# AHupuJR/REFID

Measured on AMD Instinct MI355X. Metric: interpolated frames/sec (train step) GoPro 256x256 11+1, higher is better.
Workload: dtype f32

## Files before the change

refid_amd/csrc/conv_split.hip:

```cpp
#include "common.h"
#include "conv_args.h"
#include "conv_epilogue.h"
#include "conv_planes.h"

#ifndef REFID_SPLIT_ABLATE
#define REFID_SPLIT_ABLATE 0
#endif

namespace {

constexpr int F16_TGT = 8;
constexpr int F16_SLACK = 6;
constexpr int F16_E0 = F16_TGT + 1;
constexpr int TW = 32;
constexpr int KC = 8;
constexpr int NTH = 256;
__device__ __forceinline__ int cdiv_dev(int a, int b) { return (a + b - 1) / b; }

#ifdef REFID_SPLIT_TRACE
__device__ unsigned long long* g_split_trace = nullptr;
__device__ unsigned long long* g_split_ktrace = nullptr;
__device__ int g_split_ktrace_wg = -1;
#define SPLIT_STAMP(slot)                                                                    \
    do {                                                                                     \
        if (g_split_trace && threadIdx.x == 0) g_split_trace[(size_t)blockIdx.x * 8 + (slot)] = wall_clock64(); \
    } while (0)
#define SPLIT_KSTAMP(ch, slot)                                                               \
    do {                                                                                     \
        if (ktrace && (threadIdx.x & 63) == 0)                                               \
            g_split_ktrace[(((threadIdx.x >> 6) * 64 + ((ch) & 63)) * 8) + (slot)] = wall_clock64(); \
    } while (0)
#else
#define SPLIT_STAMP(slot) do {} while (0)
#define SPLIT_KSTAMP(ch, slot) do {} while (0)
#endif

template <int MT_, int NT_, int PL_, int KS_, int MODE_, bool F16_ = false>
struct SCfg {
    static constexpr int MT = MT_, NT = NT_, PL = PL_, KS = KS_;
    static constexpr int MODE = MODE_;
    static constexpr bool F16 = F16_;
    static constexpr int TH = 4 * MT, BN = 32 * NT;
    static constexpr int HWD = (MODE == 1) ? TW + 1 : TW + 2;
    static constexpr int NTAP = (MODE == 0) ? 10 : 4;
    static constexpr int NSTEP = NTAP / 2;
    static constexpr int HP = ((MODE == 1) ? TH + 1 : TH + 2) * HWD;
    static constexpr int A_SLOTS = HP;
    static constexpr int B_SLOTS = NTAP * BN;
    static constexpr int A_ITEMS = (A_SLOTS + NTH - 1) / NTH;
    static constexpr int B_ITEMS = (PL * B_SLOTS + NTH - 1) / NTH;
    static constexpr int C4 = BN / 4;
    static constexpr int XS = C4 + 1;
    static constexpr int LDS_LOOP = KS * PL * (A_SLOTS + B_SLOTS) * 16 + (F16 ? 16 : 0);
    static constexpr int LDS_EPI = 4 * 32 * XS * 16;
    static constexpr int LDS_BYTES = LDS_LOOP > LDS_EPI ? LDS_LOOP : LDS_EPI;
};

template <int MT, int NT, int PL, int KS, int MODE, bool F16 = false>
__global__ __launch_bounds__(NTH, 2) void conv_split_kernel(const ConvKArgs a) {
    using C = SCfg<MT, NT, PL, KS, MODE, F16>;
    static_assert(!F16 || PL == 2, "the fp16 form has two planes");
    constexpr int HP = C::HP, BN = C::BN, HWD = C::HWD, NTAP = C::NTAP, NSTEP = C::NSTEP;
    static_assert(MODE != 1 || KS == 2, "MODE 1: a stage = the two column positions of a block");
    extern __shared__ __attribute__((aligned(16))) char smem[];
    f32x4* sA = reinterpret_cast<f32x4*>(smem);
    f32x4* sB = sA + KS * PL * C::A_SLOTS;
    float* sM = reinterpret_cast<float*>(sB + KS * PL * C::B_SLOTS);

    const int tid = threadIdx.x;
    const int lane = tid & 63, wave = tid >> 6;
    const int li = lane & 31, kh = lane >> 5;

    const int xcd = blockIdx.x & 7, slot = blockIdx.x >> 3;
    int bt = (slot / a.ncot) * 8 + xcd;
    if (bt >= a.tilesX * a.tilesY * a.N) return;
    const int n0 = (slot % a.ncot) * BN;
    const int tx = bt % a.tilesX; bt /= a.tilesX;
    const int ty = bt % a.tilesY;
    const int n = bt / a.tilesY;
    const int oy0 = ty * C::TH, ox0 = tx * TW;
    SPLIT_STAMP(0);
#ifdef REFID_SPLIT_TRACE
    const bool ktrace = g_split_ktrace && (int)blockIdx.x == g_split_ktrace_wg;
    if (g_split_trace && tid == 0) {
        unsigned hw, xcc;
        asm volatile("s_getreg_b32 %0, hwreg(HW_REG_HW_ID)" : "=s"(hw));
        asm volatile("s_getreg_b32 %0, hwreg(HW_REG_XCC_ID)" : "=s"(xcc));
        g_split_trace[(size_t)blockIdx.x * 8 + 7] = ((unsigned long long)xcc << 32) | hw;
    }
#endif

    const int limA = (int)min((long long)a.N * a.H * a.W * a.ldA * 4, 0x7fffffffLL);
    const int limB = a.inB ? (int)min((long long)a.N * a.H * a.W * a.ldB * 4, 0x7fffffffLL) : 0;
    const int wChunk = PL * NTAP * a.CoutPad * 16;
    const int nsub = cdiv_dev(a.Ctot, KC) * (MODE == 1 ? 4 : 1);
    const int cls = (MODE == 2) ? blockIdx.y : 0;
    const int py = cls >> 1, px = cls & 1;
    const __amdgpu_buffer_rsrc_t rsW = __builtin_amdgcn_make_buffer_rsrc(
        reinterpret_cast<char*>(const_cast<float*>(a.w)) + (F16 ? PACK_HEADER_BYTES : 0) + (long long)cls * nsub * wChunk, 0,
        (int)min((long long)nsub * wChunk, 0x7fffffffLL), 0x00020000);
    const int eW = F16 ? *reinterpret_cast<const int*>(a.w) : 0;
    int eRef = F16_E0;
    int voA[C::A_ITEMS], voB[C::A_ITEMS], vo1x[2][MODE == 1 ? C::A_ITEMS : 1];
#pragma unroll
    for (int it = 0; it < C::A_ITEMS; ++it) {
        const int hp = tid + it * NTH;
        if constexpr (MODE == 1) {
            const int r0 = 2 * (oy0 + hp / HWD) - 1, c0 = 2 * (ox0 + hp % HWD) - 1;
#pragma unroll
            for (int sy = 0; sy < 2; ++sy)
#pragma unroll
                for (int sx = 0; sx < 2; ++sx) {
                    const int iy = r0 + sy, ix = c0 + sx;
                    const bool ok = hp < HP && iy >= 0 && iy < a.H && ix >= 0 && ix < a.W;
                    const int vo = ok ? ((n * a.H + iy) * a.W + ix) * a.ldA * 4 : OOB;
                    if (sx == 0) (sy ? voB[it] : voA[it]) = vo;
                    else vo1x[sy][it] = vo;
                }
        } else {
            const int iy = oy0 - 1 + hp / HWD, ix = ox0 - 1 + hp % HWD;
            const bool ok = hp < HP && iy >= 0 && iy < a.H && ix >= 0 && ix < a.W;
            const int pix = (n * a.H + iy) * a.W + ix;
            voA[it] = ok ? pix * a.ldA * 4 : OOB;
            voB[it] = ok ? pix * a.ldB * 4 : OOB;
        }
    }
    int voW[C::B_ITEMS];
#pragma unroll
    for (int it = 0; it < C::B_ITEMS; ++it) {
        const int s = tid + it * NTH;
        const int co = s % BN, r = s / BN;
        const int row = a.coBase + n0 + co;
        voW[it] = (s < PL * C::B_SLOTS && row < a.CoutPad) ? (r * a.CoutPad + row) * 16 : OOB;
    }

    f32x4 ra[KS][C::A_ITEMS][2], rb[KS][C::B_ITEMS];
    constexpr int NLD = 2 * C::A_ITEMS + C::B_ITEMS;
    auto load_part = [&](int chReal, int part) {
        const int ch = REFID_SPLIT_ABLATE == 3 ? 0 : chReal;
#pragma unroll
        for (int sub = 0; sub < KS; ++sub) {
            const int c0 = (MODE == 1 ? (ch >> 1) : (ch * KS + sub)) * KC;
            const bool fromA = MODE != 0 || c0 < a.Ca;
            const bool cok = c0 < a.Ctot;
            const int soff = (fromA ? c0 : c0 - a.Ca) * 4;
            const bool sy1 = MODE == 1 && (ch & 1);
            const __amdgpu_buffer_rsrc_t rs = __builtin_amdgcn_make_buffer_rsrc(
                const_cast<float*>(fromA ? a.inA : a.inB), 0, fromA ? limA : limB, 0x00020000);
#pragma unroll
            for (int i = 0; i < NLD; ++i) {
                if ((sub * NLD + i) * NSTEP / NLD != part && part >= 0) continue;
                if (i < 2 * C::A_ITEMS) {
                    const int it = i >> 1;
                    int vo;
                    if constexpr (MODE == 1) vo = sub == 0 ? (sy1 ? voB[it] : voA[it]) : (sy1 ? vo1x[1][it] : vo1x[0][it]);
                    else vo = fromA ? voA[it] : voB[it];
                    if (!cok) vo = OOB;
                    ra[sub][it][i & 1] = __builtin_bit_cast(f32x4, __builtin_amdgcn_raw_buffer_load_b128(rs, vo, soff + 16 * (i & 1), 0));
                } else {
                    const int it = i - 2 * C::A_ITEMS;
                    int vo = voW[it];
                    if constexpr (MODE == 2) vo |= (ch * KS + sub < nsub) ? 0 : OOB;
                    rb[sub][it] = __builtin_bit_cast(
                        f32x4, __builtin_amdgcn_raw_buffer_load_b128(rsW, vo, (ch * KS + sub) * wChunk, 0));
                }
            }
        }
    };
    auto load_chunk = [&](int ch) { load_part(ch, -1); };
    auto post_max = [&]() {
        float tm = 0.f;
#pragma unroll
        for (int sub = 0; sub < KS; ++sub)
#pragma unroll
            for (int it = 0; it < C::A_ITEMS; ++it)
#pragma unroll
                for (int h = 0; h < 2; ++h) {
                    const f32x4 v = ra[sub][it][h];
                    tm = fmaxf(fmaxf(tm, fmaxf(fabsf(v[0]), fabsf(v[1]))), fmaxf(fabsf(v[2]), fabsf(v[3])));
                }
#pragma unroll
        for (int o = 32; o >= 1; o >>= 1) tm = fmaxf(tm, __shfl_xor(tm, o));
        if (lane == 0) sM[wave] = tm;
    };
    f32x16 acc[MT][NT];
    auto stage_scale = [&]() -> float {
        const f32x4 m4 = *reinterpret_cast<const f32x4*>(sM);
        const int eb = (int)(__float_as_uint(fmaxf(fmaxf(m4[0], m4[1]), fmaxf(m4[2], m4[3]))) >> 23);
        if (eb > eRef + F16_SLACK) {
            const int fe = 127 + eRef - eb;
            const float f = fe >= 1 ? __uint_as_float((unsigned)fe << 23) : 0.f;
#pragma unroll
            for (int m = 0; m < MT; ++m)
#pragma unroll
                for (int nn = 0; nn < NT; ++nn)
#pragma unroll
                    for (int r = 0; r < 16; ++r) acc[m][nn][r] *= f;
            eRef = eb;
        }
        return __uint_as_float((unsigned)(F16_TGT + 254 - eRef) << 23);
    };
    auto store_chunk = [&](float sc = 1.f) {
#pragma unroll
        for (int sub = 0; sub < KS; ++sub) {
#pragma unroll
            for (int it = 0; it < C::A_ITEMS; ++it) {
                const int hp = tid + it * NTH;
                f32x4 pl[PL];
                if (REFID_SPLIT_ABLATE == 2) { pl[0] = ra[sub][it][0]; if constexpr (PL >= 2) pl[1] = ra[sub][it][1]; if constexpr (PL == 3) pl[2] = ra[sub][it][0]; }
                else if constexpr (F16) split8h(ra[sub][it][0] * sc, ra[sub][it][1] * sc, pl);
                else split8<PL>(ra[sub][it][0], ra[sub][it][1], pl);
                if (hp < HP) {
#pragma unroll
                    for (int p = 0; p < PL; ++p) sA[(sub * PL + p) * HP + hp] = pl[p];
                }
            }
#pragma unroll
            for (int it = 0; it < C::B_ITEMS; ++it) {
                const int s = tid + it * NTH;
                if (s < PL * C::B_SLOTS) sB[sub * PL * C::B_SLOTS + s] = rb[sub][it];
            }
        }
    };

#pragma unroll
    for (int m = 0; m < MT; ++m)
#pragma unroll
        for (int nn = 0; nn < NT; ++nn)
#pragma unroll
            for (int r = 0; r < 16; ++r) acc[m][nn][r] = 0.f;

    constexpr int TERMS = (PL == 3) ? 6 : (PL == 2 ? 3 : 1);
    constexpr int TA[6] = {0, 0, 1, 0, 2, 1};
    constexpr int TB[6] = {0, 1, 0, 2, 0, 1};

    int aoff[NSTEP];
#pragma unroll
    for (int j = 0; j < NSTEP; ++j) {
        if (MODE == 0) {
            const int t = min(2 * j + kh, 8);
            aoff[j] = (wave * MT + t / 3) * HWD + (t % 3) + li;
        } else if (MODE == 1) {
            aoff[j] = (wave * MT + j) * HWD + kh + li;
        } else {
            const int dy = (j == 0) ? 1 : (py ? 2 : 0);
            const int dx = (kh == 0) ? 1 : (px ? 2 : 0);
            aoff[j] = (wave * MT + dy) * HWD + dx + li;
        }
    }
    const f32x4* pB = sB + kh * BN + li;

    load_chunk(0);
    if constexpr (F16) {
        post_max();
        __syncthreads();
        store_chunk(stage_scale());
    } else {
        store_chunk();
    }
    __syncthreads();
    SPLIT_STAMP(1);

    for (int ch = 0; ch < ((REFID_SPLIT_ABLATE == 5 || REFID_SPLIT_ABLATE == 7) ? 0 : a.nchunks); ++ch) {
        const bool more = ch + 1 < a.nchunks;
        SPLIT_KSTAMP(ch, 0);
        SPLIT_KSTAMP(ch, 1);
#pragma unroll
        for (int sj = 0; sj < NSTEP * KS; ++sj) {
            const int sub = sj / NSTEP, j = sj % NSTEP;
            if (more && REFID_SPLIT_ABLATE != 4) load_part(ch + 1, sj);
            f32x4 af[PL][MT], bf[PL][NT];
#pragma unroll
            for (int p = 0; p < PL; ++p) {
#pragma unroll
                for (int m = 0; m < MT; ++m)
                    af[p][m] = REFID_SPLIT_ABLATE == 8 ? ra[0][0][m & 1] : sA[(sub * PL + p) * C::A_SLOTS + m * HWD + aoff[j]];
#pragma unroll
                for (int nn = 0; nn < NT; ++nn)
                    bf[p][nn] = REFID_SPLIT_ABLATE == 8 ? rb[0][0] : pB[((sub * PL + p) * NTAP + 2 * j) * BN + nn * 32];
            }
#pragma unroll
            for (int e = 0; e < (REFID_SPLIT_ABLATE == 1 ? 0 : TERMS); ++e)
#pragma unroll
                for (int m = 0; m < MT; ++m)
#pragma unroll
                    for (int nn = 0; nn < NT; ++nn) {
                        if constexpr (F16)
                            acc[m][nn] = __builtin_amdgcn_mfma_f32_32x32x16_f16(
                                __builtin_bit_cast(f16x8, bf[TB[e]][nn]), __builtin_bit_cast(f16x8, af[TA[e]][m]),
                                acc[m][nn], 0, 0, 0);
                        else
                            acc[m][nn] = __builtin_amdgcn_mfma_f32_32x32x16_bf16(
                                __builtin_bit_cast(bf16x8, bf[TB[e]][nn]), __builtin_bit_cast(bf16x8, af[TA[e]][m]),
                                acc[m][nn], 0, 0, 0);
                    }
            __builtin_amdgcn_sched_barrier(0);
        }
        SPLIT_KSTAMP(ch, 2);
        if constexpr (F16) {
            if (more) post_max();
        }
        __syncthreads();
        SPLIT_KSTAMP(ch, 3);
#ifdef REFID_SPLIT_TRACE
        __builtin_amdgcn_s_waitcnt(0x0F70);
#endif
        SPLIT_KSTAMP(ch, 4);
        if (more) {
            if constexpr (F16) store_chunk(stage_scale());
            else store_chunk();
            SPLIT_KSTAMP(ch, 5);
            __syncthreads();
        }
        SPLIT_KSTAMP(ch, 6);
    }
    SPLIT_STAMP(2);

    constexpr int C4 = C::C4, XS = C::XS;
    constexpr int EIT = (32 * C4) / 64;
    auto opix = [&](int oy, int ox) -> long long {
        if (MODE == 2) return (long long)(n * 2 * a.Ho + 2 * oy + py) * (2 * a.Wo) + 2 * ox + px;
        return (long long)(n * a.Ho + oy) * a.Wo + ox;
    };
    f32x4* ex = reinterpret_cast<f32x4*>(smem) + wave * (32 * XS);
#pragma unroll
    for (int m = 0; m < MT; ++m) {
        const int oy = oy0 + wave * MT + m;
        f32x4 pres[EIT], pmask[EIT];
        const bool pre = a.vecOK && (a.res != nullptr || a.mask != nullptr) && REFID_SPLIT_ABLATE != 6 && REFID_SPLIT_ABLATE != 7;
        if (pre) {
#pragma unroll
            for (int it = 0; it < EIT; ++it) {
                const int f = it * 64 + lane;
                const int c4 = f % C4, px = f / C4;
                const int ox = ox0 + px, j0 = n0 + c4 * 4;
                const bool ok = oy < a.Ho && ox < a.Wo && j0 + 3 < a.Cout;
                const long long op = opix(oy, ox);
                pres[it] = f32x4{0.f, 0.f, 0.f, 0.f};
                pmask[it] = f32x4{1.f, 1.f, 1.f, 1.f};
                if (ok && a.res) pres[it] = *reinterpret_cast<const f32x4*>(a.res + op * a.ldR + j0);
                if (ok && a.mask) pmask[it] = *reinterpret_cast<const f32x4*>(a.mask + op * a.ldM + j0);
            }
        }
#pragma unroll
        for (int nn = 0; nn < NT; ++nn)
#pragma unroll
            for (int g = 0; g < 4; ++g) {
                f32x4 v;
#pragma unroll
                for (int k = 0; k < 4; ++k) {
                    v[k] = acc[m][nn][4 * g + k];
                    if constexpr (F16) v[k] = ldexpf(v[k], eRef - 127 - F16_TGT - eW);
                }
                ex[li * XS + nn * 8 + 2 * g + kh] = v;
            }
#pragma unroll
        for (int it = 0; it < EIT; ++it) {
            const int f = it * 64 + lane;
            const int c4 = f % C4, px = f / C4;
            const int ox = ox0 + px, j0 = n0 + c4 * 4;
            f32x4 v = ex[px * XS + c4];
            if (oy >= a.Ho || ox >= a.Wo || j0 >= a.Cout) continue;
            const long long op = opix(oy, ox);
            const bool vec = a.vecOK && (j0 + 3 < a.Cout);
            v += epi_bias4(a, a.coBase + j0, j0, vec);
            epi_pre(a, v);
            if (REFID_SPLIT_ABLATE == 6 || REFID_SPLIT_ABLATE == 7) {
                if (v[0] == 12345.678f) a.out[op * a.ldO + j0] = v[1];
                continue;
            }
            epi_tail(a, v, j0, vec, EpiAtOp{op, j0}, true, pres[it], pmask[it]);
        }
    }
    SPLIT_STAMP(3);
}

template <int MT, int NT, int PL, int KS, int MODE, bool F16 = false>
int launch_split(const ConvKArgs& ka, hipStream_t st) {
    using C = SCfg<MT, NT, PL, KS, MODE, F16>;
    static std::atomic<unsigned long long> attr_done{0};
    if (int rc = refid_lds_attr_once(attr_done, &conv_split_kernel<MT, NT, PL, KS, MODE, F16>, C::LDS_BYTES, "conv_split")) return rc;
    ConvKArgs a = ka;
    a.tilesX = cdiv(a.Wo, TW);
    a.tilesY = cdiv(a.Ho, C::TH);
    a.nchunks = (MODE == 1) ? 2 * cdiv(a.Ctot, KC) : cdiv(a.Ctot, KC * KS);
    a.ncot = cdiv(a.Cout, C::BN);
    const int tiles = a.tilesX * a.tilesY * a.N;
    dim3 grid(cdiv(tiles, 8) * 8 * a.ncot, MODE == 2 ? 4 : 1);
    hipLaunchKernelGGL((conv_split_kernel<MT, NT, PL, KS, MODE, F16>), grid, dim3(NTH), C::LDS_BYTES, st, a);
    REFID_LAUNCH_CHECK("conv_split");
    return 0;
}

template <int PL, int MODE, bool F16 = false>
int launch_split_pl(const ConvKArgs& a, bool wide, bool tall, hipStream_t st) {
    constexpr int KS = (MODE == 0) ? 1 : 2;
    if (wide) return tall ? launch_split<2, 2, PL, KS, MODE, F16>(a, st) : launch_split<1, 2, PL, KS, MODE, F16>(a, st);
    return tall ? launch_split<2, 1, PL, KS, MODE, F16>(a, st) : launch_split<1, 1, PL, KS, MODE, F16>(a, st);
}

}

#ifdef REFID_SPLIT_TRACE
extern "C" int refid_split_trace_set(unsigned long long* wg_stamps, unsigned long long* k_stamps, int wg) {
    if (hipMemcpyToSymbol(HIP_SYMBOL(g_split_trace), &wg_stamps, sizeof(wg_stamps)) != hipSuccess) return 1;
    if (hipMemcpyToSymbol(HIP_SYMBOL(g_split_ktrace), &k_stamps, sizeof(k_stamps)) != hipSuccess) return 1;
    return hipMemcpyToSymbol(HIP_SYMBOL(g_split_ktrace_wg), &wg, sizeof(wg)) != hipSuccess;
}
#endif

bool refid_split3x3_eligible(const ConvKArgs& a) {
    const long long lim = 0x7fffffffLL;
    return a.Ctot % 8 == 0 && (a.inB == nullptr || a.Ca % KC == 0) &&
           (long long)a.N * a.H * a.W * a.ldA * 4 < lim && (!a.inB || (long long)a.N * a.H * a.W * a.ldB * 4 < lim) &&
           a.ldA % 4 == 0 && (!a.inB || a.ldB % 4 == 0);
}

int refid_launch_split3x3(const ConvKArgs& a, int terms, int mode, int cus, int split_mode, hipStream_t st) {
    REFID_CHECK(terms == 1 || terms == 3 || terms == 6 || (terms == 19 && mode != 0),
                "conv2d: split tile takes 1, 3 or 6 product terms, or 19 (three fp16 products; 4x4 stride 2 and its input "
                "gradient only) (got %d)", terms);
    REFID_CHECK(terms != 19 || (reinterpret_cast<uintptr_t>(a.w) & 15) == 0, "conv2d: the fp16 split packing must be 16-byte aligned");
    REFID_CHECK(refid_split3x3_eligible(a) && (mode == 0 || a.inB == nullptr),
                "conv2d: split tile needs channel counts that are multiples of 8, tensors below 2 GiB and, for the stride-2 "
                "modes, a single source");
    {
        const long long planes = terms == 6 ? 3 : ((terms == 3 || terms == 19) ? 2 : 1);
        const long long wbytes = (long long)cdiv(a.Ctot, KC) * (mode == 1 ? 4 : 1) * planes * (mode == 0 ? 10 : 4) * a.CoutPad * 16;
        REFID_CHECK(wbytes < 0x7fffffffLL, "conv2d: packed weights too large for the split tile's 32-bit offsets");
    }
    const bool wide = a.Cout > 32;
    const bool per_sample = split_mode == 1 || terms == 19;
    const int wg8 = cdiv(a.Wo, TW) * cdiv(a.Ho, 8) * (per_sample ? 8 : a.N) * cdiv(a.Cout, wide ? 64 : 32) * (mode == 2 ? 4 : 1);
    const bool tall = wg8 >= 2 * cus;
#define SPLIT_DISPATCH(PLN)                                                          \
    (mode == 0 ? launch_split_pl<PLN, 0>(a, wide, tall, st)                          \
               : (mode == 1 ? launch_split_pl<PLN, 1>(a, wide, tall, st) : launch_split_pl<PLN, 2>(a, wide, tall, st)))
    if (terms == 19) return mode == 1 ? launch_split_pl<2, 1, true>(a, wide, tall, st) : launch_split_pl<2, 2, true>(a, wide, tall, st);
    if (terms == 6) return SPLIT_DISPATCH(3);
    if (terms == 3) return SPLIT_DISPATCH(2);
    return SPLIT_DISPATCH(1);
#undef SPLIT_DISPATCH
}
```

Measured before the change: 547.3.

## Add line-wise 16-channel input loading path for stride-2 split conv modes

Adds an LN variant of the split-precision conv kernel for the stride-2 modes. Four adjacent threads each load a 4-channel quad of one pixel, so a stage covers 16 contiguous channels per pixel instead of per-thread 8-channel strips. This is meant to make global loads more coalesced and cut per-thread offset registers. The variant changes the LDS layout with padded A sub-buffers and uses a higher launch-bounds occupancy hint for small tiles. It is enabled by default through launch_split_down, with REFID_DOWN_LINES=0 as an opt-out, and adds the risk of register spills and new indexing bugs.

```diff
diff --git a/refid_amd/csrc/conv_split.hip b/refid_amd/csrc/conv_split.hip
--- a/refid_amd/csrc/conv_split.hip
+++ b/refid_amd/csrc/conv_split.hip
@@ -35,11 +35,12 @@
 #define SPLIT_KSTAMP(ch, slot) do {} while (0)
 #endif
 
-template <int MT_, int NT_, int PL_, int KS_, int MODE_, bool F16_ = false>
+template <int MT_, int NT_, int PL_, int KS_, int MODE_, bool F16_ = false, bool LN_ = false>
 struct SCfg {
     static constexpr int MT = MT_, NT = NT_, PL = PL_, KS = KS_;
     static constexpr int MODE = MODE_;
     static constexpr bool F16 = F16_;
+    static constexpr bool LN = LN_;
     static constexpr int TH = 4 * MT, BN = 32 * NT;
     static constexpr int HWD = (MODE == 1) ? TW + 1 : TW + 2;
     static constexpr int NTAP = (MODE == 0) ? 10 : 4;
@@ -51,20 +52,22 @@
     static constexpr int B_ITEMS = (PL * B_SLOTS + NTH - 1) / NTH;
     static constexpr int C4 = BN / 4;
     static constexpr int XS = C4 + 1;
-    static constexpr int LDS_LOOP = KS * PL * (A_SLOTS + B_SLOTS) * 16 + (F16 ? 16 : 0);
+    static constexpr int A_SUB = LN ? PL * A_SLOTS + ((12 - (PL * A_SLOTS) % 8) % 8) : PL * A_SLOTS;
+    static constexpr int LDS_LOOP = KS * (A_SUB + PL * B_SLOTS) * 16 + (F16 ? 16 : 0);
     static constexpr int LDS_EPI = 4 * 32 * XS * 16;
     static constexpr int LDS_BYTES = LDS_LOOP > LDS_EPI ? LDS_LOOP : LDS_EPI;
 };
 
-template <int MT, int NT, int PL, int KS, int MODE, bool F16 = false>
-__global__ __launch_bounds__(NTH, 2) void conv_split_kernel(const ConvKArgs a) {
-    using C = SCfg<MT, NT, PL, KS, MODE, F16>;
+template <int MT, int NT, int PL, int KS, int MODE, bool F16 = false, bool LN = false>
+__global__ __launch_bounds__(NTH, (LN && MT * NT == 1 && PL <= 2 && !F16) ? 7 : 2) void conv_split_kernel(const ConvKArgs a) {
+    using C = SCfg<MT, NT, PL, KS, MODE, F16, LN>;
     static_assert(!F16 || PL == 2, "the fp16 form has two planes");
+    static_assert(!LN || (MODE != 0 && KS == 2 && C::A_ITEMS <= 2), "lines: the stride-2 modes, 16 channels per stage, <= 8 loads");
     constexpr int HP = C::HP, BN = C::BN, HWD = C::HWD, NTAP = C::NTAP, NSTEP = C::NSTEP;
     static_assert(MODE != 1 || KS == 2, "MODE 1: a stage = the two column positions of a block");
     extern __shared__ __attribute__((aligned(16))) char smem[];
     f32x4* sA = reinterpret_cast<f32x4*>(smem);
-    f32x4* sB = sA + KS * PL * C::A_SLOTS;
+    f32x4* sB = sA + KS * C::A_SUB;
     float* sM = reinterpret_cast<float*>(sB + KS * PL * C::B_SLOTS);
 
     const int tid = threadIdx.x;
@@ -102,8 +105,31 @@
     const int eW = F16 ? *reinterpret_cast<const int*>(a.w) : 0;
     int eRef = F16_E0;
     int voA[C::A_ITEMS], voB[C::A_ITEMS], vo1x[2][MODE == 1 ? C::A_ITEMS : 1];
-#pragma unroll
-    for (int it = 0; it < C::A_ITEMS; ++it) {
+    constexpr int NQ = LN ? 4 * C::A_ITEMS : 1;
+    const int q = tid & 3;
+    int voL[NQ];
+    unsigned okL = 0;
+    if constexpr (LN) {
+#pragma unroll
+        for (int k = 0; k < NQ; ++k) {
+            const int hp = k * 64 + (tid >> 2);
+            if constexpr (MODE == 1) {
+                const int r0 = 2 * (oy0 + hp / HWD) - 1, c0 = 2 * (ox0 + hp % HWD) - 1;
+                voL[k] = (int)((((unsigned)(n * a.H + r0) * (unsigned)a.W + (unsigned)c0) * (unsigned)a.ldA + (unsigned)(q * 4)) * 4u);
+#pragma unroll
+                for (int s = 0; s < 4; ++s) {
+                    const int iy = r0 + (s >> 1), ix = c0 + (s & 1);
+                    if (hp < HP && iy >= 0 && iy < a.H && ix >= 0 && ix < a.W) okL |= 1u << (4 * k + s);
+                }
+            } else {
+                const int iy = oy0 - 1 + hp / HWD, ix = ox0 - 1 + hp % HWD;
+                const bool ok = hp < HP && iy >= 0 && iy < a.H && ix >= 0 && ix < a.W;
+                voL[k] = ok ? (((n * a.H + iy) * a.W + ix) * a.ldA + q * 4) * 4 : OOB;
+            }
+        }
+    }
+#pragma unroll
+    for (int it = 0; it < (LN ? 0 : C::A_ITEMS); ++it) {
         const int hp = tid + it * NTH;
         if constexpr (MODE == 1) {
             const int r0 = 2 * (oy0 + hp / HWD) - 1, c0 = 2 * (ox0 + hp % HWD) - 1;
@@ -135,8 +161,37 @@
     }
 
     f32x4 ra[KS][C::A_ITEMS][2], rb[KS][C::B_ITEMS];
+    f32x4 raL[NQ];
     constexpr int NLD = 2 * C::A_ITEMS + C::B_ITEMS;
+    const int nG = cdiv_dev(a.Ctot, 2 * KC);
+    int lnG = 0, lnPos = 0;
+    auto load_part_ln = [&](int part) {
+        const int G = REFID_SPLIT_ABLATE == 3 ? 0 : lnG, pos = REFID_SPLIT_ABLATE == 3 ? 0 : lnPos;
+        const __amdgpu_buffer_rsrc_t rs = __builtin_amdgcn_make_buffer_rsrc(const_cast<float*>(a.inA), 0, limA, 0x00020000);
+        const int dpos = MODE == 1 ? ((pos >> 1) * a.W + (pos & 1)) * a.ldA * 4 : 0;
+        const int cm = (G * 2 * KC + (q >> 1) * KC < a.Ctot) ? 0 : OOB;
+#pragma unroll
+        for (int sub = 0; sub < KS; ++sub) {
+            const int kidx = MODE == 1 ? (2 * G + sub) * 4 + pos : 2 * G + sub;
+#pragma unroll
+            for (int i = 0; i < NLD; ++i) {
+                if ((sub * NLD + i) * NSTEP / NLD != part && part >= 0) continue;
+                if (i < 2 * C::A_ITEMS) {
+                    const int k = sub * 2 * C::A_ITEMS + i;
+                    int vo;
+                    if constexpr (MODE == 1) vo = (voL[k] + dpos) | ((int)((okL >> (4 * k + pos)) & 1u) - 1) | cm;
+                    else vo = voL[k] | cm;
+                    raL[k] = __builtin_bit_cast(f32x4, __builtin_amdgcn_raw_buffer_load_b128(rs, vo, G * 2 * KC * 4, 0));
+                } else {
+                    const int it = i - 2 * C::A_ITEMS;
+                    const int vo = voW[it] | (kidx < nsub ? 0 : OOB);
+                    rb[sub][it] = __builtin_bit_cast(f32x4, __builtin_amdgcn_raw_buffer_load_b128(rsW, vo, kidx * wChunk, 0));
+                }
+            }
+        }
+    };
     auto load_part = [&](int chReal, int part) {
+        if constexpr (LN) { load_part_ln(part); return; }
         const int ch = REFID_SPLIT_ABLATE == 3 ? 0 : chReal;
 #pragma unroll
         for (int sub = 0; sub < KS; ++sub) {
@@ -170,8 +225,15 @@
     auto load_chunk = [&](int ch) { load_part(ch, -1); };
     auto post_max = [&]() {
         float tm = 0.f;
-#pragma unroll
-        for (int sub = 0; sub < KS; ++sub)
+        if constexpr (LN) {
+#pragma unroll
+            for (int k = 0; k < NQ; ++k) {
+                const f32x4 v = raL[k];
+                tm = fmaxf(fmaxf(tm, fmaxf(fabsf(v[0]), fabsf(v[1]))), fmaxf(fabsf(v[2]), fabsf(v[3])));
+            }
+        }
+#pragma unroll
+        for (int sub = 0; sub < (LN ? 0 : KS); ++sub)
 #pragma unroll
             for (int it = 0; it < C::A_ITEMS; ++it)
 #pragma unroll
@@ -201,10 +263,26 @@
         return __uint_as_float((unsigned)(F16_TGT + 254 - eRef) << 23);
     };
     auto store_chunk = [&](float sc = 1.f) {
+        if constexpr (LN) {
+            f32x2* hA = reinterpret_cast<f32x2*>(sA + (q >> 1) * C::A_SUB) + (q & 1);
+            const f32x4 zero = {0.f, 0.f, 0.f, 0.f};
+#pragma unroll
+            for (int k = 0; k < NQ; ++k) {
+                const int hp = k * 64 + (tid >> 2);
+                f32x4 pl[PL];
+                if (REFID_SPLIT_ABLATE == 2) { pl[0] = raL[k]; if constexpr (PL >= 2) pl[1] = raL[k]; if constexpr (PL == 3) pl[2] = raL[k]; }
+                else if constexpr (F16) split8h(raL[k] * sc, zero, pl);
+                else split8<PL>(raL[k], zero, pl);
+                if (hp < HP) {
+#pragma unroll
+                    for (int p = 0; p < PL; ++p) hA[(p * C::A_SLOTS + hp) * 2] = f32x2{pl[p][0], pl[p][1]};
+                }
+            }
+        }
 #pragma unroll
         for (int sub = 0; sub < KS; ++sub) {
 #pragma unroll
-            for (int it = 0; it < C::A_ITEMS; ++it) {
+            for (int it = 0; it < (LN ? 0 : C::A_ITEMS); ++it) {
                 const int hp = tid + it * NTH;
                 f32x4 pl[PL];
                 if (REFID_SPLIT_ABLATE == 2) { pl[0] = ra[sub][it][0]; if constexpr (PL >= 2) pl[1] = ra[sub][it][1]; if constexpr (PL == 3) pl[2] = ra[sub][it][0]; }
@@ -263,6 +341,9 @@
 
     for (int ch = 0; ch < ((REFID_SPLIT_ABLATE == 5 || REFID_SPLIT_ABLATE == 7) ? 0 : a.nchunks); ++ch) {
         const bool more = ch + 1 < a.nchunks;
+        if constexpr (LN) {
+            if (++lnG == nG && MODE == 1) { lnG = 0; ++lnPos; }
+        }
         SPLIT_KSTAMP(ch, 0);
         SPLIT_KSTAMP(ch, 1);
 #pragma unroll
@@ -274,7 +355,8 @@
             for (int p = 0; p < PL; ++p) {
 #pragma unroll
                 for (int m = 0; m < MT; ++m)
-                    af[p][m] = REFID_SPLIT_ABLATE == 8 ? ra[0][0][m & 1] : sA[(sub * PL + p) * C::A_SLOTS + m * HWD + aoff[j]];
+                    af[p][m] = REFID_SPLIT_ABLATE == 8 ? (LN ? raL[m & 1] : ra[0][0][m & 1])
+                                                       : sA[sub * C::A_SUB + p * C::A_SLOTS + m * HWD + aoff[j]];
 #pragma unroll
                 for (int nn = 0; nn < NT; ++nn)
                     bf[p][nn] = REFID_SPLIT_ABLATE == 8 ? rb[0][0] : pB[((sub * PL + p) * NTAP + 2 * j) * BN + nn * 32];
@@ -375,28 +457,37 @@
     SPLIT_STAMP(3);
 }
 
-template <int MT, int NT, int PL, int KS, int MODE, bool F16 = false>
+template <int MT, int NT, int PL, int KS, int MODE, bool F16 = false, bool LN = false>
 int launch_split(const ConvKArgs& ka, hipStream_t st) {
-    using C = SCfg<MT, NT, PL, KS, MODE, F16>;
+    using C = SCfg<MT, NT, PL, KS, MODE, F16, LN>;
     static std::atomic<unsigned long long> attr_done{0};
-    if (int rc = refid_lds_attr_once(attr_done, &conv_split_kernel<MT, NT, PL, KS, MODE, F16>, C::LDS_BYTES, "conv_split")) return rc;
+    if (int rc = refid_lds_attr_once(attr_done, &conv_split_kernel<MT, NT, PL, KS, MODE, F16, LN>, C::LDS_BYTES, "conv_split")) return rc;
     ConvKArgs a = ka;
     a.tilesX = cdiv(a.Wo, TW);
     a.tilesY = cdiv(a.Ho, C::TH);
-    a.nchunks = (MODE == 1) ? 2 * cdiv(a.Ctot, KC) : cdiv(a.Ctot, KC * KS);
+    a.nchunks = (MODE == 1) ? (LN ? 4 * cdiv(a.Ctot, 2 * KC) : 2 * cdiv(a.Ctot, KC)) : cdiv(a.Ctot, KC * KS);
     a.ncot = cdiv(a.Cout, C::BN);
     const int tiles = a.tilesX * a.tilesY * a.N;
     dim3 grid(cdiv(tiles, 8) * 8 * a.ncot, MODE == 2 ? 4 : 1);
-    hipLaunchKernelGGL((conv_split_kernel<MT, NT, PL, KS, MODE, F16>), grid, dim3(NTH), C::LDS_BYTES, st, a);
+    hipLaunchKernelGGL((conv_split_kernel<MT, NT, PL, KS, MODE, F16, LN>), grid, dim3(NTH), C::LDS_BYTES, st, a);
     REFID_LAUNCH_CHECK("conv_split");
     return 0;
 }
 
-template <int PL, int MODE, bool F16 = false>
+template <int PL, int MODE, bool F16 = false, bool LN = false>
 int launch_split_pl(const ConvKArgs& a, bool wide, bool tall, hipStream_t st) {
     constexpr int KS = (MODE == 0) ? 1 : 2;
-    if (wide) return tall ? launch_split<2, 2, PL, KS, MODE, F16>(a, st) : launch_split<1, 2, PL, KS, MODE, F16>(a, st);
-    return tall ? launch_split<2, 1, PL, KS, MODE, F16>(a, st) : launch_split<1, 1, PL, KS, MODE, F16>(a, st);
+    if (wide) return tall ? launch_split<2, 2, PL, KS, MODE, F16, LN>(a, st) : launch_split<1, 2, PL, KS, MODE, F16, LN>(a, st);
+    return tall ? launch_split<2, 1, PL, KS, MODE, F16, LN>(a, st) : launch_split<1, 1, PL, KS, MODE, F16, LN>(a, st);
+}
+
+template <int PL, int MODE, bool F16 = false>
+int launch_split_down(const ConvKArgs& a, bool wide, bool tall, hipStream_t st) {
+    static const bool lines = []() { const char* e = getenv("REFID_DOWN_LINES"); return !(e && e[0] == '0'); }();
+    if constexpr (!(F16 && MODE == 1)) {
+        if (lines && (MODE == 2 || a.Ctot <= 64)) return launch_split_pl<PL, MODE, F16, true>(a, wide, tall, st);
+    }
+    return launch_split_pl<PL, MODE, F16, false>(a, wide, tall, st);
 }
 
 }
@@ -435,8 +526,8 @@
     const bool tall = wg8 >= 2 * cus;
 #define SPLIT_DISPATCH(PLN)                                                          \
     (mode == 0 ? launch_split_pl<PLN, 0>(a, wide, tall, st)                          \
-               : (mode == 1 ? launch_split_pl<PLN, 1>(a, wide, tall, st) : launch_split_pl<PLN, 2>(a, wide, tall, st)))
-    if (terms == 19) return mode == 1 ? launch_split_pl<2, 1, true>(a, wide, tall, st) : launch_split_pl<2, 2, true>(a, wide, tall, st);
+               : (mode == 1 ? launch_split_down<PLN, 1>(a, wide, tall, st) : launch_split_down<PLN, 2>(a, wide, tall, st)))
+    if (terms == 19) return mode == 1 ? launch_split_down<2, 1, true>(a, wide, tall, st) : launch_split_down<2, 2, true>(a, wide, tall, st);
     if (terms == 6) return SPLIT_DISPATCH(3);
     if (terms == 3) return SPLIT_DISPATCH(2);
     return SPLIT_DISPATCH(1);
```

Result: no change. 549.6 (median of 6 runs) (+0.4%).
